# zengxiaofei/HapHiC

Hardware: NVIDIA H100
Metric: hic_pairs_per_sec_matrix_build (higher is better)
Workload: dtype int32 counts / fp32 matrix

## Files before the change

### haphic_b200/csrc/hh_common.cuh

```cuda
#pragma once

#include <cuda_runtime.h>
#include <stdint.h>
#include <stdio.h>
#include <stdarg.h>
#include <string.h>
#include <new>
#include <vector>

#include "../../include/haphic_b200.h"

void hh_set_error(const char* fmt, ...);

#define HH_CUDA(expr)                                                                         \
    do {                                                                                      \
        cudaError_t _e = (expr);                                                              \
        if (_e != cudaSuccess) {                                                              \
            hh_set_error("%s:%d: %s failed: %s", __FILE__, __LINE__, #expr, cudaGetErrorString(_e)); \
            return (_e == cudaErrorMemoryAllocation) ? HH_ERR_NOMEM : HH_ERR_CUDA;            \
        }                                                                                     \
    } while (0)

#define HH_CHECK(expr)                                                                        \
    do {                                                                                      \
        int _rc = (expr);                                                                     \
        if (_rc != HH_OK) return _rc;                                                         \
    } while (0)

#define HH_REQUIRE(cond, code, ...)                                                           \
    do {                                                                                      \
        if (!(cond)) {                                                                        \
            hh_set_error(__VA_ARGS__);                                                        \
            return (code);                                                                    \
        }                                                                                     \
    } while (0)

#define HH_LAUNCH(ctx, kernel, grid, block, smem, ...)                                        \
    do {                                                                                      \
        kernel<<<(grid), (block), (smem), (ctx)->stream>>>(__VA_ARGS__);                      \
        (ctx)->launches++;                                                                    \
        HH_CUDA(cudaGetLastError());                                                          \
    } while (0)

struct hh_ctx {
    int device;
    int sm_count;
    size_t smem_optin;
    size_t l2_bytes;
    cudaStream_t stream;
    int64_t launches;
    uint64_t* h_scratch;
    uint64_t* d_scratch;
    struct ws_block {
        void* p;
        size_t bytes;
        bool used;
        uint64_t tick;
    };
    std::vector<ws_block>* ws;
    uint64_t ws_tick;
};

void* hh_ws_alloc_bytes(hh_ctx* ctx, size_t bytes);
bool hh_ws_release(hh_ctx* ctx, void* p);
void hh_ws_free_ptr(hh_ctx* ctx, void* p);
template <typename T>
static inline int hh_ws_alloc(hh_ctx* ctx, T** p, size_t count) {
    *p = reinterpret_cast<T*>(hh_ws_alloc_bytes(ctx, (count ? count : 1) * sizeof(T)));
    return *p ? HH_OK : HH_ERR_NOMEM;
}
template <typename T>
static inline void hh_ws_free(hh_ctx* ctx, T*& p) {
    if (p) hh_ws_free_ptr(ctx, (void*)p);
    p = nullptr;
}

extern thread_local hh_ctx* hh_tls_ctx;
struct hh_scope {
    hh_ctx* prev;
    explicit hh_scope(hh_ctx* c) : prev(hh_tls_ctx) {
        hh_tls_ctx = c;
        if (c) cudaSetDevice(c->device);
    }
    ~hh_scope() { hh_tls_ctx = prev; }
};

#define HH_WS_MIN ((size_t)32 << 20)
template <typename T>
static inline int hh_dmalloc(T** p, size_t count) {
    *p = nullptr;
    if (count == 0) count = 1;
    if (hh_tls_ctx && count * sizeof(T) >= HH_WS_MIN) {
        *p = reinterpret_cast<T*>(hh_ws_alloc_bytes(hh_tls_ctx, count * sizeof(T)));
        return *p ? HH_OK : HH_ERR_NOMEM;
    }
    cudaError_t e = hh_tls_ctx ? cudaMallocAsync((void**)p, count * sizeof(T), hh_tls_ctx->stream)
                               : cudaMalloc((void**)p, count * sizeof(T));
    if (e != cudaSuccess) {
        hh_set_error("cudaMalloc of %zu bytes failed: %s", count * sizeof(T), cudaGetErrorString(e));
        cudaGetLastError();
        return HH_ERR_NOMEM;
    }
    return HH_OK;
}
template <typename T>
static inline void hh_dfree(T*& p) {
    if (p) {
        if (hh_ws_release(hh_tls_ctx, (void*)p)) {
        } else if (hh_tls_ctx) {
            cudaFreeAsync((void*)p, hh_tls_ctx->stream);
        } else {
            cudaFree((void*)p);
        }
    }
    p = nullptr;
}

#define HH_FULL_MASK 0xffffffffu

__device__ __forceinline__ int hh_lane() { return threadIdx.x & 31; }
__device__ __forceinline__ int hh_warp() { return threadIdx.x >> 5; }

__device__ __forceinline__ double hh_warp_sum(double v) {
#pragma unroll
    for (int o = 16; o > 0; o >>= 1) v += __shfl_xor_sync(HH_FULL_MASK, v, o);
    return v;
}
__device__ __forceinline__ int hh_warp_sum(int v) {
#pragma unroll
    for (int o = 16; o > 0; o >>= 1) v += __shfl_xor_sync(HH_FULL_MASK, v, o);
    return v;
}
__device__ __forceinline__ unsigned long long hh_warp_sum(unsigned long long v) {
#pragma unroll
    for (int o = 16; o > 0; o >>= 1) v += __shfl_xor_sync(HH_FULL_MASK, v, o);
    return v;
}
template <typename T>
__device__ __forceinline__ T hh_warp_incl_scan(T v) {
#pragma unroll
    for (int o = 1; o < 32; o <<= 1) {
        const T t = __shfl_up_sync(HH_FULL_MASK, v, o);
        if (hh_lane() >= o) v += t;
    }
    return v;
}
__device__ __forceinline__ float hh_warp_max(float v) {
#pragma unroll
    for (int o = 16; o > 0; o >>= 1) v = fmaxf(v, __shfl_xor_sync(HH_FULL_MASK, v, o));
    return v;
}

__device__ __forceinline__ int4 hh_ld_stream(const int4* p) {
    int4 r;
    asm volatile("ld.global.nc.L1::no_allocate.v4.s32 {%0, %1, %2, %3}, [%4];"
                 : "=r"(r.x), "=r"(r.y), "=r"(r.z), "=r"(r.w)
                 : "l"(p));
    return r;
}
__device__ __forceinline__ unsigned long long hh_ld_stream_u64(const unsigned long long* p) {
    unsigned long long r;
    asm volatile("ld.global.nc.L1::no_allocate.u64 %0, [%1];" : "=l"(r) : "l"(p));
    return r;
}
__device__ __forceinline__ float4 hh_ld_stream_f4(const float4* p) {
    float4 r;
    asm volatile("ld.global.nc.L1::no_allocate.v4.f32 {%0, %1, %2, %3}, [%4];"
                 : "=f"(r.x), "=f"(r.y), "=f"(r.z), "=f"(r.w)
                 : "l"(p));
    return r;
}

template <typename K>
static inline int hh_resident_grid(hh_ctx* ctx, K kernel, int threads, size_t smem, int* grid) {
    int per_sm = 0;
    HH_CUDA(cudaOccupancyMaxActiveBlocksPerMultiprocessor(&per_sm, kernel, threads, smem));
    HH_REQUIRE(per_sm > 0, HH_ERR_CUDA, "a kernel of %d threads and %zu bytes of shared memory does not fit an SM", threads, smem);
    *grid = ctx->sm_count * per_sm;
    return HH_OK;
}

__global__ void hh_k_scan_small(const int* __restrict__ in, int64_t* __restrict__ out, int n);
int hh_exclusive_scan_i32(hh_ctx* ctx, const int* d_in, int64_t* d_out, int n);
```

### haphic_b200/csrc/hh_links.cu

```cuda
#include "hh_common.cuh"
#include "hh_internal.cuh"
#include <cub/cub.cuh>
#include <stdlib.h>
#include <algorithm>
#include <vector>

#define HH_EMPTY_KEY 0xFFFFFFFFFFFFFFFFull
#define HH_NONE32 0xFFFFFFFFu

struct __align__(32) hh_slot {
    uint32_t first_full, first_flank, full, flank, ht, th, tt, pad;
};

struct hh_partset {
    void* buf;
    bool narrow;
    unsigned long long* cursor;
    uint64_t pcap;
    int64_t sized_for, sent;
};

struct hh_links {
    hh_ctx* ctx;
    int32_t n_ctg;
// ... 41 lines not shown
    int32_t* d_deg;
    int64_t n_pass;
    uint64_t gen;
    bool ix_valid;
    uint64_t ix_gen;
    int ix_normalize;
    double ix_w;
    std::vector<uint8_t> ix_keep;
    std::vector<int32_t> ix_hap;
    unsigned long long* d_ul_key = nullptr;
    int32_t* d_ul_slot = nullptr;
    int64_t n_ul = 0;
};

__device__ __forceinline__ uint64_t hh_mix64(uint64_t k) {
    k ^= k >> 33;
    k *= 0xff51afd7ed558ccdull;
    k ^= k >> 33;
    k *= 0xc4ceb9fe1a85ec53ull;
    k ^= k >> 33;
    return k;
}

__device__ __forceinline__ uint64_t hh_probe_insert(uint64_t* __restrict__ keys, uint64_t cap, uint64_t key, bool* inserted) {
    const uint64_t mask = cap - 1;
    uint64_t slot = hh_mix64(key) & mask;
    *inserted = false;
    for (uint64_t probes = 0; probes < cap; ++probes) {
        uint64_t k = *((volatile uint64_t*)(keys + slot));
        if (k == key) return slot;
        if (k == HH_EMPTY_KEY) {
            unsigned long long prev = atomicCAS((unsigned long long*)(keys + slot), (unsigned long long)HH_EMPTY_KEY,
                                                (unsigned long long)key);
            if (prev == HH_EMPTY_KEY) {
                *inserted = true;
                return slot;
            }
            if (prev == key) return slot;
        }
        slot = (slot + 1) & mask;
    }
    return cap;
}

__global__ void hh_k_links_init(uint64_t* __restrict__ keys, hh_slot* __restrict__ vals, uint64_t cap) {
    const uint64_t stride = (uint64_t)gridDim.x * blockDim.x;
    for (uint64_t s = (uint64_t)blockIdx.x * blockDim.x + threadIdx.x; s < cap; s += stride) {
        keys[s] = HH_EMPTY_KEY;
        uint4* v = reinterpret_cast<uint4*>(vals + s);
        v[0] = make_uint4(HH_NONE32, HH_NONE32, 0u, 0u);
        v[1] = make_uint4(0u, 0u, 0u, 0u);
    }
}

#define HH_F_FLANK 1u
#define HH_F_TI 2u
#define HH_F_TJ 4u

struct hh_pair {
    int a, b;
    unsigned flags;
};

__device__ __forceinline__ uint64_t hh_pair_key(int a, int b) { return ((uint64_t)(uint32_t)a << 32) | (uint64_t)(uint32_t)b; }

__device__ __forceinline__ void hh_swap_ends(int& a, int& b, int& pa, int& pb) {
    int t = a; a = b; b = t;
    t = pa; pa = pb; pb = t;
}

__device__ __forceinline__ void hh_pair_flags(int a, int b, int pa, int pb, const int32_t* __restrict__ ctg_len,
                                              const uint8_t* __restrict__ in_nx, int64_t flank_bp, hh_pair* out) {
    const int64_t coord_i = (int64_t)pa + 1, coord_j = (int64_t)pb + 1;
    const int64_t li = ctg_len[a], lj = ctg_len[b];
    const bool fi = (flank_bp == 0) || (coord_i <= flank_bp) || (coord_i > li - flank_bp);
    const bool fj = (flank_bp == 0) || (coord_j <= flank_bp) || (coord_j > lj - flank_bp);
    out->a = a;
    out->b = b;
    out->flags = ((fi && fj && in_nx[a] && in_nx[b]) ? HH_F_FLANK : 0u)
                 | ((coord_i * 2 > li) ? HH_F_TI : 0u) | ((coord_j * 2 > lj) ? HH_F_TJ : 0u);
}

__device__ __forceinline__ bool hh_classify_contig(int4 r, int32_t n_ctg, const int32_t* __restrict__ ctg_len,
                                                   const int32_t* __restrict__ name_rank, const uint8_t* __restrict__ in_nx,
                                                   int64_t flank_bp, hh_pair* out) {
    int a = r.x, b = r.z, pa = r.y, pb = r.w;
    if (a == b || (unsigned)a >= (unsigned)n_ctg || (unsigned)b >= (unsigned)n_ctg) return false;
    if (name_rank[a] > name_rank[b]) hh_swap_ends(a, b, pa, pb);
    hh_pair_flags(a, b, pa, pb, ctg_len, in_nx, flank_bp, out);
    return true;
}

__device__ __forceinline__ int64_t hh_floor_div(int64_t x, int64_t d) { return x >= 0 ? x / d : -((-x + d - 1) / d); }

__device__ __forceinline__ bool hh_to_bin(int& f, int& p, int nbins, int64_t bin_size) {
    const int64_t nb = ((int64_t)p + 1 + bin_size - 1) / bin_size;
    const bool exists = p >= 0 && nb >= 1 && nb <= (int64_t)nbins;
    f += (int)(nb - 1);
    p = (int)((int64_t)p - (nb - 1) * bin_size);
    return exists;
}

__device__ __forceinline__ bool hh_classify_frag(int4 r, int32_t n_src, const int32_t* __restrict__ src_rank,
                                                 const int32_t* __restrict__ fbase, int64_t bin_size, const int32_t* __restrict__ ctg_len,
                                                 const int32_t* __restrict__ name_rank, const uint8_t* __restrict__ in_nx,
                                                 int64_t flank_bp, uint32_t idx, unsigned long long* __restrict__ counters,
                                                 hh_pair* out) {
    int a = r.x, b = r.z, pa = r.y, pb = r.w;
    if ((unsigned)a >= (unsigned)n_src || (unsigned)b >= (unsigned)n_src) return false;
    if (a == b && fbase[a + 1] - fbase[a] <= 1) return false;
    if (src_rank[a] > src_rank[b] || (a == b && pa > pb)) hh_swap_ends(a, b, pa, pb);
    int fa = fbase[a], fb = fbase[b];
    const int na = fbase[a + 1] - fa, nb = fbase[b + 1] - fb;
    if (a == b && hh_floor_div((int64_t)pa, bin_size) == hh_floor_div((int64_t)pb, bin_size)) return false;
    bool bad = false;
    if (na > 1) bad = !hh_to_bin(fa, pa, na, bin_size);
    if (nb > 1) bad = !hh_to_bin(fb, pb, nb, bin_size) || bad;
    if (bad) {
        atomicAdd(counters + 5, 1ull);
        atomicMax(counters + 6, (unsigned long long)idx + 1ull);
        return false;
    }
    if (fa == fb) return false;
    if ((na > 1 || nb > 1) && name_rank[fa] > name_rank[fb]) hh_swap_ends(fa, fb, pa, pb);
    hh_pair_flags(fa, fb, pa, pb, ctg_len, in_nx, flank_bp, out);
    return true;
}

struct hh_group {
    bool leader;
    uint32_t first_all, first_flank;
    unsigned full, flank, ht, th, tt;
};

__device__ __forceinline__ hh_group hh_warp_fold(bool ok, uint64_t key, uint32_t idx, unsigned flags) {
    const int lane = threadIdx.x & 31;
    if (!ok) key = HH_EMPTY_KEY - 1 - (uint64_t)lane;
    const unsigned peers = __match_any_sync(HH_FULL_MASK, key);
    const bool fl = ok && (flags & HH_F_FLANK), ti = (flags & HH_F_TI) != 0, tj = (flags & HH_F_TJ) != 0;
    hh_group g;
    g.first_all = __reduce_min_sync(peers, ok ? idx : HH_NONE32);
    g.first_flank = __reduce_min_sync(peers, fl ? idx : HH_NONE32);
    const unsigned b_fl = __ballot_sync(HH_FULL_MASK, fl);
    const unsigned b_ht = __ballot_sync(HH_FULL_MASK, ok && !ti && tj);
    const unsigned b_th = __ballot_sync(HH_FULL_MASK, ok && ti && !tj);
    const unsigned b_tt = __ballot_sync(HH_FULL_MASK, ok && ti && tj);
    g.leader = ok && lane == (__ffs(peers) - 1);
    g.full = __popc(peers);
    g.flank = __popc(peers & b_fl);
    g.ht = __popc(peers & b_ht);
    g.th = __popc(peers & b_th);
    g.tt = __popc(peers & b_tt);
    return g;
}

__device__ __forceinline__ void hh_slot_update(hh_slot* v, const hh_group& g) {
    atomicAdd(&v->full, g.full);
    atomicMin(&v->first_full, g.first_all);
    if (g.flank) {
        atomicAdd(&v->flank, g.flank);
        atomicMin(&v->first_flank, g.first_flank);
    }
    if (g.ht) atomicAdd(&v->ht, g.ht);
    if (g.th) atomicAdd(&v->th, g.th);
    if (g.tt) atomicAdd(&v->tt, g.tt);
}

__device__ __forceinline__ void hh_entry_store(uint32_t* __restrict__ o, uint64_t key, uint32_t full, uint32_t flank, uint32_t first_full,
                                               uint32_t first_flank, uint32_t ht, uint32_t th, uint32_t tt) {
    o[HH_E_I] = (uint32_t)(key >> 32);
    o[HH_E_J] = (uint32_t)key;
    o[HH_E_FULL] = full;
    o[HH_E_FLANK] = flank;
    o[HH_E_FIRST_FULL] = first_full;
    o[HH_E_FIRST_FLANK] = first_flank;
    o[HH_E_HT] = ht;
    o[HH_E_TH] = th;
    o[HH_E_TT] = tt;
}

__device__ __forceinline__ void hh_entry_store(uint32_t* __restrict__ o, uint64_t key, uint4 v0, uint4 v1) {
    hh_entry_store(o, key, v0.z, v0.w, v0.x, v0.y, v1.x, v1.y, v1.z);
}

__device__ __forceinline__ unsigned int hh_block_rank(unsigned int cnt, unsigned int* s_wtot, unsigned int* total) {
    const int lane = threadIdx.x & 31, wv = threadIdx.x >> 5;
    unsigned int incl = cnt;
#pragma unroll
    for (int o = 1; o < 32; o <<= 1) {
        const unsigned int t = __shfl_up_sync(HH_FULL_MASK, incl, o);
        if (lane >= o) incl += t;
    }
    __syncthreads();
    if (lane == 31) s_wtot[wv] = incl;
    __syncthreads();
    unsigned int before = 0, all = 0;
#pragma unroll
    for (int k = 0; k < 8; ++k) {
        const unsigned int t = s_wtot[k];
        before += (k < wv) ? t : 0u;
        all += t;
    }
    *total = all;
    return before + incl - cnt;
}

__global__ void __launch_bounds__(256)
hh_k_links_insert(const int4* __restrict__ rec, int64_t n_rec, uint32_t stream_off, int32_t n_ctg,
                  const int32_t* __restrict__ ctg_len, const int32_t* __restrict__ name_rank,
                  const uint8_t* __restrict__ in_nx, int64_t flank_bp, uint64_t* __restrict__ keys,
                  hh_slot* __restrict__ vals, uint64_t cap, unsigned long long* __restrict__ ctg_links,
                  unsigned long long* __restrict__ counters, const int32_t* __restrict__ src_rank,
                  const int32_t* __restrict__ fbase, int64_t bin_size, int32_t n_src, const uint32_t* __restrict__ pos) {
    __shared__ unsigned int s_new, s_used, s_over;
    if (threadIdx.x == 0) {
        s_new = 0;
        s_used = 0;
        s_over = 0;
    }
    __syncthreads();
    const int lane = threadIdx.x & 31;
    const int64_t stride = (int64_t)gridDim.x * blockDim.x;
    unsigned int my_new = 0, my_used = 0;
    for (int64_t i0 = (int64_t)blockIdx.x * blockDim.x + (threadIdx.x - lane); i0 < n_rec; i0 += stride) {
        const int64_t i = i0 + lane;
        bool ok = i < n_rec;
        hh_pair p = {0, 0, 0u};
        uint32_t idx = HH_NONE32;
        if (ok) {
            const int4 r = hh_ld_stream(rec + i);
            idx = pos ? pos[i] : stream_off + (uint32_t)i;
            ok = fbase == nullptr ? hh_classify_contig(r, n_ctg, ctg_len, name_rank, in_nx, flank_bp, &p)
                                  : hh_classify_frag(r, n_src, src_rank, fbase, bin_size, ctg_len, name_rank, in_nx, flank_bp, idx,
                                                     counters, &p);
        }
        if (ok) my_used++;
        const uint64_t key = hh_pair_key(p.a, p.b);
        const hh_group g = hh_warp_fold(ok, key, idx, p.flags);
        if (g.leader) {
            bool inserted;
            const uint64_t slot = hh_probe_insert(keys, cap, key, &inserted);
            if (slot >= cap) {
                s_over = 1;
            } else {
                if (inserted) my_new++;
                hh_slot_update(vals + slot, g);
                if (g.flank) {
                    atomicAdd(ctg_links + p.a, (unsigned long long)g.flank);
                    atomicAdd(ctg_links + p.b, (unsigned long long)g.flank);
                }
            }
        }
    }
    if (my_new) atomicAdd(&s_new, my_new);
    if (my_used) atomicAdd(&s_used, my_used);
    __syncthreads();
    if (threadIdx.x == 0) {
        if (s_new) atomicAdd(counters + 0, (unsigned long long)s_new);
        if (s_used) atomicAdd(counters + 1, (unsigned long long)s_used);
        if (s_over) atomicExch(counters + 2, 1ull);
    }
}

#define HH_PART_TILE 4096
#define HH_PART_MAX 1024

#define HH_NREC_KBITS 16
#define HH_NREC_ZBITS 29
#define HH_NREC_ZEND (1ll << HH_NREC_ZBITS)

struct __align__(8) hh_nrec {
    unsigned long long v;
};

__device__ __forceinline__ int4 hh_ld_rec(const int4* p) { return hh_ld_stream(p); }
__device__ __forceinline__ hh_nrec hh_ld_rec(const hh_nrec* p) { return hh_nrec{hh_ld_stream_u64(&p->v)}; }

__device__ __forceinline__ uint32_t hh_rec_i(int4 r, int) { return (uint32_t)r.x; }
__device__ __forceinline__ uint32_t hh_rec_j(int4 r, int) { return (uint32_t)r.y; }
__device__ __forceinline__ uint32_t hh_rec_z(int4 r) { return (uint32_t)r.z; }
__device__ __forceinline__ unsigned hh_rec_flags(int4 r) { return (unsigned)r.w & 7u; }
__device__ __forceinline__ uint32_t hh_rec_i(hh_nrec r, int kbits) { return (uint32_t)(r.v >> 32) >> kbits; }
__device__ __forceinline__ uint32_t hh_rec_j(hh_nrec r, int kbits) { return (uint32_t)(r.v >> 32) & ((1u << kbits) - 1u); }
__device__ __forceinline__ uint32_t hh_rec_z(hh_nrec r) { return (uint32_t)r.v & (uint32_t)(HH_NREC_ZEND - 1); }
__device__ __forceinline__ unsigned hh_rec_flags(hh_nrec r) { return (uint32_t)r.v >> HH_NREC_ZBITS; }

__device__ __forceinline__ hh_nrec hh_nrec_make(uint32_t i, uint32_t j, uint32_t z, unsigned flags, int kbits) {
    return hh_nrec{((unsigned long long)((i << kbits) | j) << 32) | ((unsigned long long)flags << HH_NREC_ZBITS) | z};
}

__device__ __forceinline__ void hh_rec_put(int4* d, int4 s, int) { *d = s; }
__device__ __forceinline__ void hh_rec_put(hh_nrec* d, hh_nrec s, int) { *d = s; }
__device__ __forceinline__ void hh_rec_put(int4* d, hh_nrec s, int kbits) {
    *d = make_int4((int)hh_rec_i(s, kbits), (int)hh_rec_j(s, kbits), (int)hh_rec_z(s), (int)hh_rec_flags(s));
}
__device__ __forceinline__ void hh_rec_put(hh_nrec* d, int4 s, int kbits) {
    *d = hh_nrec_make(hh_rec_i(s, kbits), hh_rec_j(s, kbits), hh_rec_z(s), hh_rec_flags(s), kbits);
}

__device__ __forceinline__ void hh_rec_set_z(int4* r, uint32_t z) { r->z = (int)z; }
__device__ __forceinline__ void hh_rec_set_z(hh_nrec* r, uint32_t z) { r->v = (r->v & ~(unsigned long long)(HH_NREC_ZEND - 1)) | z; }

#define HH_STAGE_SMEM ((size_t)HH_PART_TILE * sizeof(int4))

__device__ __forceinline__ unsigned int hh_tile_scan(unsigned int* c, int n, unsigned int* s_wtot) {
    const int lane = threadIdx.x & 31, wv = threadIdx.x >> 5;
    const int per = (n + 511) >> 9, lo = threadIdx.x * per;
    __syncthreads();
    unsigned int sum = 0;
    for (int k = 0; k < per; ++k)
        if (lo + k < n) sum += c[lo + k];
    unsigned int incl = sum;
#pragma unroll
    for (int o = 1; o < 32; o <<= 1) {
        const unsigned int t = __shfl_up_sync(HH_FULL_MASK, incl, o);
        if (lane >= o) incl += t;
    }
    if (lane == 31) s_wtot[wv] = incl;
    __syncthreads();
    unsigned int run = incl - sum, all = 0;
#pragma unroll
    for (int k = 0; k < 16; ++k) {
        const unsigned int t = s_wtot[k];
        run += (k < wv) ? t : 0u;
        all += t;
    }
    for (int k = 0; k < per; ++k) {
        if (lo + k < n) {
            const unsigned int t = c[lo + k];
            c[lo + k] = run;
            run += t;
        }
    }
    __syncthreads();
    return all;
}

template <typename R>
__device__ __forceinline__ uint32_t hh_bucket_of(R r, int bucket_log, int kbits) {
    return (uint32_t)(hh_mix64(hh_pair_key((int)hh_rec_i(r, kbits), (int)hh_rec_j(r, kbits))) >> (64 - bucket_log));
}

__device__ __forceinline__ void hh_part_rec(int4* o, const hh_pair& pr, uint32_t z, unsigned p, int) {
    *o = make_int4(pr.a, pr.b, (int)z, (int)(pr.flags | (p << 8)));
}
__device__ __forceinline__ void hh_part_rec(hh_nrec* o, const hh_pair& pr, uint32_t z, unsigned, int kbits) {
    *o = hh_nrec_make((uint32_t)pr.a, (uint32_t)pr.b, z, pr.flags, kbits);
}
__device__ __forceinline__ unsigned hh_part_of(int4 r, int, int) { return (unsigned)r.w >> 8; }
__device__ __forceinline__ unsigned hh_part_of(hh_nrec r, int npart_log, int kbits) { return hh_bucket_of(r, npart_log, kbits); }

template <typename R>
__host__ __device__ constexpr int hh_scatter_tile() { return (int)(HH_STAGE_SMEM / sizeof(R)); }

template <typename R>
__global__ void __launch_bounds__(512, 2)
hh_k_part_scatter(const int4* __restrict__ rec, int64_t n_rec, uint32_t stream_off, int32_t n_ctg, const int32_t* __restrict__ ctg_len,
                  const int32_t* __restrict__ name_rank, const uint8_t* __restrict__ in_nx, int64_t flank_bp, int npart_log, int kbits,
                  R* __restrict__ pbuf, uint64_t pcap, unsigned long long* __restrict__ cursor, int4* __restrict__ spill,
                  uint64_t spill_cap, unsigned long long* __restrict__ spill_cursor, unsigned long long* __restrict__ counters) {
    constexpr int TILE = hh_scatter_tile<R>(), ITEMS = TILE / 512;
    extern __shared__ int4 s_stage_mem[];
    R* s_stage = reinterpret_cast<R*>(s_stage_mem);
    __shared__ unsigned int s_cnt[HH_PART_MAX];
    __shared__ unsigned long long s_base[HH_PART_MAX];
    __shared__ unsigned int s_wtot[16];
    __shared__ unsigned int s_used;
    const int npart = 1 << npart_log;
    const int64_t tiles = (n_rec + TILE - 1) / TILE;
    unsigned int my_used = 0;
    if (threadIdx.x == 0) s_used = 0;
    for (int64_t t = blockIdx.x; t < tiles; t += gridDim.x) {
        for (int k = threadIdx.x; k < npart; k += 512) s_cnt[k] = 0;
        __syncthreads();
        R out[ITEMS];
        uint32_t live = 0;
#pragma unroll
        for (int k = 0; k < ITEMS; ++k) {
            const int64_t i = t * TILE + (int64_t)k * 512 + threadIdx.x;
            if (i < n_rec) {
                hh_pair pr;
                if (hh_classify_contig(hh_ld_stream(rec + i), n_ctg, ctg_len, name_rank, in_nx, flank_bp, &pr)) {
                    const unsigned p = (unsigned)(hh_mix64(hh_pair_key(pr.a, pr.b)) >> (64 - npart_log));
                    hh_part_rec(&out[k], pr, (p << 13) | atomicAdd(&s_cnt[p], 1u), p, kbits);
                    live |= 1u << k;
                    my_used++;
                }
            }
        }
        __syncthreads();
        for (int k = threadIdx.x; k < npart; k += 512)
            if (s_cnt[k]) s_base[k] = atomicAdd(cursor + k, (unsigned long long)s_cnt[k]);
        const unsigned int n_tile = hh_tile_scan(s_cnt, npart, s_wtot);
#pragma unroll
        for (int k = 0; k < ITEMS; ++k) {
            if (!((live >> k) & 1u)) continue;
            const uint32_t at = hh_rec_z(out[k]);
            hh_rec_set_z(&out[k], stream_off + (uint32_t)(t * TILE + k * 512 + threadIdx.x));
            s_stage[s_cnt[at >> 13] + (at & 0x1FFFu)] = out[k];
        }
        __syncthreads();
        for (unsigned int e = threadIdx.x; e < n_tile; e += 512) {
            const R r = s_stage[e];
            const unsigned int p = hh_part_of(r, npart_log, kbits);
            const unsigned long long q = s_base[p] + (e - s_cnt[p]);
            if (q < pcap) {
                pbuf[(size_t)p * (size_t)pcap + (size_t)q] = r;
            } else {
                const unsigned long long sq = atomicAdd(spill_cursor, 1ull);
                if (sq < spill_cap) hh_rec_put(spill + sq, r, kbits);
                else atomicExch(counters + 2, 3ull);
            }
        }
        __syncthreads();
    }
    my_used = (unsigned)hh_warp_sum((int)my_used);
    if ((threadIdx.x & 31) == 0 && my_used) atomicAdd(&s_used, my_used);
    __syncthreads();
    if (threadIdx.x == 0 && s_used) atomicAdd(counters + 1, (unsigned long long)s_used);
}

#define HH_AGG_MEAN 2048
#define HH_SUB_MAX_LOG 12
#define HH_AGG_SLOTS 2048
#define HH_AGG_LIST (HH_AGG_SLOTS / 4 * 3)
#define HH_AGG_THREADS 256
#define HH_AGG_HOT 32

template <typename R>
__global__ void __launch_bounds__(512)
hh_k_part_hist(const R* __restrict__ pbuf, uint64_t pcap, const unsigned long long* __restrict__ cursor, int npart_log, int kbits,
               int64_t tpr, const int4* __restrict__ spill, int64_t n_spill, int bucket_log, unsigned int* __restrict__ bcnt) {
    constexpr int TILE = HH_PART_TILE, ITEMS = TILE / 512;
    __shared__ unsigned int s_cnt[1 << HH_SUB_MAX_LOG];
    const int sub_log = bucket_log - npart_log, nsub = 1 << sub_log;
    const int64_t region_tiles = ((int64_t)1 << npart_log) * tpr;
    const int64_t tiles = region_tiles + (n_spill + HH_PART_TILE - 1) / HH_PART_TILE;
    for (int64_t t = blockIdx.x; t < tiles; t += gridDim.x) {
        if (t >= region_tiles) {
            const int64_t base = (t - region_tiles) * HH_PART_TILE;
            for (int k = threadIdx.x; k < HH_PART_TILE; k += 512)
                if (base + k < n_spill) atomicAdd(bcnt + hh_bucket_of(hh_ld_rec(spill + base + k), bucket_log, kbits), 1u);
            continue;
        }
        const int p = (int)(t / tpr);
        const uint64_t start = (uint64_t)(t % tpr) * TILE;
        const uint64_t fill = min((uint64_t)cursor[p], pcap);
        if (start >= fill) continue;
        for (int k = threadIdx.x; k < nsub; k += 512) s_cnt[k] = 0;
        __syncthreads();
        const R* reg = pbuf + (size_t)p * (size_t)pcap;
#pragma unroll
        for (int k = 0; k < ITEMS; ++k) {
            const uint64_t i = start + (uint64_t)k * 512 + threadIdx.x;
            if (i < fill) atomicAdd(&s_cnt[hh_bucket_of(hh_ld_rec(reg + i), bucket_log, kbits) & (nsub - 1)], 1u);
        }
        __syncthreads();
        for (int k = threadIdx.x; k < nsub; k += 512)
            if (s_cnt[k]) atomicAdd(bcnt + ((size_t)p << sub_log) + k, s_cnt[k]);
        __syncthreads();
    }
}

template <typename R, typename D>
__global__ void __launch_bounds__(512, 2)
hh_k_part_scatter2(const R* __restrict__ pbuf, uint64_t pcap, const unsigned long long* __restrict__ cursor, int npart_log, int kbits,
                   int64_t tpr, const int4* __restrict__ spill, int64_t n_spill, int bucket_log, const int64_t* __restrict__ boff,
                   unsigned int* __restrict__ bfill, D* __restrict__ out, uint64_t n_out, unsigned long long* __restrict__ counters) {
    constexpr int TILE = HH_PART_TILE, ITEMS = TILE / 512;
    extern __shared__ int4 s_stage_mem[];
    R* s_stage = reinterpret_cast<R*>(s_stage_mem);
    __shared__ unsigned int s_cnt[1 << HH_SUB_MAX_LOG];
    __shared__ unsigned int s_base[1 << HH_SUB_MAX_LOG];
    __shared__ unsigned int s_wtot[16];
    const int sub_log = bucket_log - npart_log, nsub = 1 << sub_log;
    const int64_t region_tiles = ((int64_t)1 << npart_log) * tpr;
    const int64_t tiles = region_tiles + (n_spill + HH_PART_TILE - 1) / HH_PART_TILE;
    for (int64_t t = blockIdx.x; t < tiles; t += gridDim.x) {
        if (t >= region_tiles) {
            const int64_t base = (t - region_tiles) * HH_PART_TILE;
            for (int k = threadIdx.x; k < HH_PART_TILE; k += 512) {
                if (base + k >= n_spill) break;
                const int4 r = hh_ld_rec(spill + base + k);
                const uint32_t b = hh_bucket_of(r, bucket_log, kbits);
                const uint64_t q = (uint64_t)boff[b] + atomicAdd(bfill + b, 1u);
                if (q < n_out) hh_rec_put(out + q, r, kbits);
                else atomicExch(counters + 2, 6ull);
            }
            continue;
        }
        const int p = (int)(t / tpr);
        const uint64_t start = (uint64_t)(t % tpr) * TILE;
        const uint64_t fill = min((uint64_t)cursor[p], pcap);
        if (start >= fill) continue;
        for (int k = threadIdx.x; k < nsub; k += 512) s_cnt[k] = 0;
        __syncthreads();
        const R* reg = pbuf + (size_t)p * (size_t)pcap;
        R r[ITEMS];
        uint32_t at[ITEMS];
#pragma unroll
        for (int k = 0; k < ITEMS; ++k) {
            const uint64_t i = start + (uint64_t)k * 512 + threadIdx.x;
            at[k] = HH_NONE32;
            if (i < fill) {
                r[k] = hh_ld_rec(reg + i);
                const uint32_t sub = hh_bucket_of(r[k], bucket_log, kbits) & (nsub - 1);
                at[k] = (sub << 16) | atomicAdd(&s_cnt[sub], 1u);
            }
        }
        __syncthreads();
        for (int k = threadIdx.x; k < nsub; k += 512)
            if (s_cnt[k]) s_base[k] = atomicAdd(bfill + ((size_t)p << sub_log) + k, s_cnt[k]);
        const unsigned int n_tile = hh_tile_scan(s_cnt, nsub, s_wtot);
#pragma unroll
        for (int k = 0; k < ITEMS; ++k)
            if (at[k] != HH_NONE32) s_stage[s_cnt[at[k] >> 16] + (at[k] & 0xFFFFu)] = r[k];
        __syncthreads();
        for (unsigned int e = threadIdx.x; e < n_tile; e += 512) {
            const R rec = s_stage[e];
            const uint32_t sub = hh_bucket_of(rec, bucket_log, kbits) & (nsub - 1);
            const size_t b = ((size_t)p << sub_log) + sub;
            const uint64_t q = (uint64_t)boff[b] + s_base[sub] + (e - s_cnt[sub]);
            if (q < n_out) hh_rec_put(out + q, rec, kbits);
            else atomicExch(counters + 2, 6ull);
        }
        __syncthreads();
    }
}

#define HH_PK_FLANK 12
#define HH_PK_HT 24
#define HH_PK_TH 36
#define HH_PK_TT 48
#define HH_PK_MASK 0xFFFull
#define HH_PK_HEAD (1ull << 63)

struct hh_run {
    unsigned long long c;
    uint32_t first_full, first_flank;
};

struct hh_run_op {
    __device__ __forceinline__ hh_run operator()(const hh_run& a, const hh_run& b) const {
        if (b.c & HH_PK_HEAD) return b;
        return hh_run{a.c + b.c, min(a.first_full, b.first_full), min(a.first_flank, b.first_flank)};
    }
};

template <typename K>
__device__ __forceinline__ int hh_lower_bound(const K* a, int n, K k) {
    int lo = 0, hi = n;
    while (lo < hi) {
        const int mid = (lo + hi) >> 1;
        if (a[mid] < k) lo = mid + 1;
        else hi = mid;
    }
    return lo;
}

template <typename K, int ITEMS>
struct hh_bc_smem {
    typedef cub::BlockRadixSort<K, HH_AGG_THREADS, ITEMS, uint32_t> sort_t;
    typedef cub::BlockScan<hh_run, HH_AGG_THREADS> run_scan_t;
    typedef cub::BlockScan<unsigned int, HH_AGG_THREADS> cnt_scan_t;
    K key[HH_AGG_LIST];
    uint32_t val[HH_E_WORDS - 2][HH_AGG_LIST];
    uint32_t z[HH_AGG_THREADS * ITEMS];
    union {
        typename sort_t::TempStorage sort;
        struct {
            K first[HH_AGG_THREADS], last[HH_AGG_THREADS];
        } edge;
        K fresh[HH_AGG_THREADS * ITEMS];
    } u;
    typename run_scan_t::TempStorage run_scan;
    typename cnt_scan_t::TempStorage cnt_scan;
    unsigned long long base;
    int bucket;
};

template <typename K, int ITEMS, typename R>
__global__ void __launch_bounds__(HH_AGG_THREADS, 3)
hh_k_bucket_count(const R* __restrict__ rec, const int64_t* __restrict__ boff, int nbuckets, uint64_t hot, int kbits,
                  uint32_t* __restrict__ compact, uint64_t compact_cap, unsigned long long* __restrict__ ctg_links,
                  unsigned long long* __restrict__ counters, unsigned long long* __restrict__ agg, uint32_t* __restrict__ fallback) {
    typedef hh_bc_smem<K, ITEMS> smem_t;
    constexpr int S = HH_AGG_THREADS * ITEMS;
    extern __shared__ __align__(16) unsigned char hh_agg_smem[];
    smem_t& sm = *reinterpret_cast<smem_t*>(hh_agg_smem);
    const int t = threadIdx.x;
    const K jmask = ((K)1 << kbits) - 1;
    const hh_run none = {HH_PK_HEAD, HH_NONE32, HH_NONE32};
    unsigned int nfl = 0, n_done = 0;
    for (;;) {
        __syncthreads();
        if (t == 0) sm.bucket = (int)atomicAdd(agg + 0, 1ull);
        __syncthreads();
        const int bk = sm.bucket;
        if (bk >= nbuckets) break;
        const int64_t lo = boff[bk], n = boff[bk + 1] - lo;
        if ((uint64_t)n > hot) {
            if (t == 0) fallback[atomicAdd(agg + 1, 1ull)] = (uint32_t)bk;
            continue;
        }
        int tsize = HH_AGG_THREADS;
        while (tsize < HH_AGG_SLOTS && (int64_t)tsize * 2 < n * 3) tsize <<= 1;
        const int limit = tsize / 4 * 3;
        int na = 0;
        bool abandon = false;
        for (int64_t c0 = 0; c0 < n; c0 += S) {
            const int m = (int)min((int64_t)S, n - c0);
            K key[ITEMS];
            uint32_t pay[ITEMS];
            __syncthreads();
#pragma unroll
            for (int q = 0; q < ITEMS; ++q) {
                const int l = q * HH_AGG_THREADS + t;
                key[q] = ~(K)0;
                pay[q] = 0;
                if (l < m) {
                    const R r = hh_ld_rec(rec + lo + c0 + l);
                    key[q] = ((K)hh_rec_i(r, kbits) << kbits) | (K)hh_rec_j(r, kbits);
                    pay[q] = (uint32_t)l | (hh_rec_flags(r) << 11);
                    sm.z[l] = hh_rec_z(r);
                }
            }
            typename smem_t::sort_t(sm.u.sort).Sort(key, pay, 0, 2 * kbits);
            __syncthreads();
            sm.u.edge.first[t] = key[0];
            sm.u.edge.last[t] = key[ITEMS - 1];
            __syncthreads();
            const K prev = t > 0 ? sm.u.edge.last[t - 1] : ~(K)0;
            const K next = t + 1 < HH_AGG_THREADS ? sm.u.edge.first[t + 1] : ~(K)0;
            auto item = [&](int q) -> hh_run {
                const int pos = t * ITEMS + q;
                if (pos >= m) return none;
                const unsigned f = (pay[q] >> 11) & 7u;
                const uint32_t z = sm.z[pay[q] & 0x7FFu];
                const bool fl = f & HH_F_FLANK, ti = f & HH_F_TI, tj = f & HH_F_TJ;
// ... 1615 lines not shown
```

### haphic_b200/csrc/hh_matrix.cu

```cuda
#include "hh_common.cuh"
#include "hh_internal.cuh"
#include <algorithm>

__global__ void hh_k_set_tail(const int32_t* __restrict__ tail, int n_tail, int n_linked, const uint8_t* __restrict__ keep,
                              int32_t* __restrict__ index, int n_ctg, int* __restrict__ err) {
    int t = blockIdx.x * blockDim.x + threadIdx.x;
    if (t >= n_tail) return;
    const int c = tail[t];
    if (c < 0 || c >= n_ctg || !keep[c] || index[c] >= 0) {
        atomicExch(err, 1);
        return;
    }
    index[c] = n_linked + t;
}

__global__ void hh_k_check_index(const int32_t* __restrict__ index, const uint8_t* __restrict__ keep, int n_ctg, int n,
                                 int* __restrict__ err) {
    int c = blockIdx.x * blockDim.x + threadIdx.x;
    if (c >= n_ctg) return;
    const int ix = index[c];
    if (keep[c] ? (ix < 0 || ix >= n) : (ix >= 0)) atomicExch(err, 2);
}

__global__ void hh_k_fill_i32(int* __restrict__ p, int v, int n) {
    int i = blockIdx.x * blockDim.x + threadIdx.x;
    if (i < n) p[i] = v;
}

__global__ void hh_k_mat_colcnt(const int32_t* __restrict__ index, const int32_t* __restrict__ deg, int n_ctg, int self_loop,
                                int* __restrict__ colcnt) {
    const int c = blockIdx.x * blockDim.x + threadIdx.x;
    if (c >= n_ctg) return;
    const int ix = index[c];
    if (ix >= 0) colcnt[ix] = deg[c] + self_loop;
}

__global__ void hh_k_mat_self_loops(int n, const int64_t* __restrict__ colptr, int32_t* __restrict__ row, float* __restrict__ val) {
    const int c = blockIdx.x * blockDim.x + threadIdx.x;
    if (c >= n) return;
    const int64_t q = colptr[c];
    row[q] = c;
    val[q] = 1.0f;
}

__global__ void hh_k_mat_scatter(const uint32_t* __restrict__ compact, int64_t nnz, const int32_t* __restrict__ index,
                                 const unsigned long long* __restrict__ ctg_tot, int normalize, const int32_t* __restrict__ hap,
                                 double w, const int32_t* __restrict__ ul_path, const int32_t* __restrict__ ul_parent,
                                 const int64_t* __restrict__ colptr, int* __restrict__ cursor,
                                 int32_t* __restrict__ row, float* __restrict__ val) {
    const int64_t stride = (int64_t)gridDim.x * blockDim.x;
    for (int64_t e = (int64_t)blockIdx.x * blockDim.x + threadIdx.x; e < nnz; e += stride) {
        const uint32_t* p = compact + e * HH_E_WORDS;
        if (p[HH_E_FLANK] == 0) continue;
        const int ii = index[p[HH_E_I]], jj = index[p[HH_E_J]];
        if (ii < 0 || jj < 0) continue;
        double x;
        if (!hh_flank_value(p, ctg_tot, normalize, hap, w, ul_path, ul_parent, &x)) continue;
        const float v = (float)x;
        int64_t q = colptr[jj] + atomicAdd(cursor + jj, 1);
        row[q] = ii;
        val[q] = v;
        q = colptr[ii] + atomicAdd(cursor + ii, 1);
        row[q] = jj;
        val[q] = v;
    }
}

static int matrix_alloc(hh_ctx* ctx, int32_t n, int64_t nnz, hh_matrix** out) {
    hh_matrix* m = new (std::nothrow) hh_matrix();
    HH_REQUIRE(m != nullptr, HH_ERR_NOMEM, "hh_matrix: out of host memory");
    memset(m, 0, sizeof(*m));
    m->ctx = ctx;
    m->n = n;
    m->nnz = nnz;
    int rc;
    if ((rc = hh_dmalloc(&m->d_colptr, (size_t)n + 1)) != HH_OK || (rc = hh_dmalloc(&m->d_row, (size_t)nnz)) != HH_OK ||
        (rc = hh_dmalloc(&m->d_val, (size_t)nnz)) != HH_OK) {
        hh_matrix_destroy(m);
        return rc;
    }
    *out = m;
    return HH_OK;
}

extern "C" int hh_matrix_from_links(hh_links* lk, const uint8_t* keep, const int32_t* tail, int32_t n_tail,
                                    int normalize_by_nlinks, int add_self_loops, hh_matrix** out) {
    return hh_matrix_from_links_phased(lk, keep, tail, n_tail, normalize_by_nlinks, add_self_loops, nullptr, 0.0, out);
}

extern "C" int hh_matrix_from_links_phased(hh_links* lk, const uint8_t* keep, const int32_t* tail, int32_t n_tail,
                                           int normalize_by_nlinks, int add_self_loops, const int32_t* hap, double w,
                                           hh_matrix** out) {
    return hh_matrix_from_links_ex(lk, keep, tail, n_tail, normalize_by_nlinks, add_self_loops, hap, w, nullptr, nullptr, out);
}

extern "C" int hh_matrix_from_links_ex(hh_links* lk, const uint8_t* keep, const int32_t* tail, int32_t n_tail, int normalize_by_nlinks,
                                       int add_self_loops, const int32_t* hap, double w, const int32_t* ul_path,
                                       const int32_t* ul_parent, hh_matrix** out) {
    HH_REQUIRE(lk && keep && out, HH_ERR_ARG, "hh_matrix_from_links: NULL argument");
    hh_scope _scope(hh_links_ctx(lk));
    HH_REQUIRE(n_tail >= 0 && (tail || n_tail == 0), HH_ERR_ARG, "hh_matrix_from_links: bad tail");
    HH_REQUIRE(!ul_path == !ul_parent, HH_ERR_ARG, "hh_matrix_from_links_ex: give both ul_path and ul_parent, or neither");
    HH_REQUIRE(hh_links_finished(lk), HH_ERR_STATE, "hh_matrix_from_links: call hh_links_finish first");
    *out = nullptr;
    hh_ctx* ctx = hh_links_ctx(lk);
    HH_CUDA(cudaSetDevice(ctx->device));
    const int n_ctg = hh_links_n_ctg(lk);
    int32_t n_linked = 0;
    HH_CHECK(hh_links_linked_index_phased(lk, keep, normalize_by_nlinks, hap, w, nullptr, &n_linked));
    const int32_t* d_hap = hh_links_hap_dev(lk);
    const int32_t* d_index = hh_links_index_dev(lk, &n_linked);
    int64_t n_pass = 0;
    const int32_t* d_deg = hh_links_degree_dev(lk, &n_pass);
    const uint8_t* d_keep = hh_links_keep_dev(lk);
    HH_REQUIRE(n_tail <= n_ctg - n_linked, HH_ERR_ARG,
               "hh_matrix_from_links: tail lists an id that is dropped, linked, repeated or out of range");
    const int n = n_linked + n_tail;
    HH_REQUIRE(n > 0, HH_ERR_ARG, "hh_matrix_from_links: empty fragment set");
    const int sl = add_self_loops ? 1 : 0;
    const int64_t nnz = 2 * n_pass + (int64_t)sl * n;
    int* d_err = reinterpret_cast<int*>(ctx->d_scratch + 10);
    int32_t* d_tail = nullptr;
    int32_t* d_ul = nullptr;
    int* d_cnt = nullptr;
    hh_matrix* m = nullptr;
    int rc = [&]() -> int {
        HH_CHECK(matrix_alloc(ctx, n, nnz, &m));
        HH_CHECK(hh_dmalloc(&m->d_index, (size_t)n_ctg));
        m->n_index = n_ctg;
        HH_CUDA(cudaMemcpyAsync(m->d_index, d_index, (size_t)n_ctg * sizeof(int32_t), cudaMemcpyDeviceToDevice, ctx->stream));
        HH_CUDA(cudaMemsetAsync(d_err, 0, sizeof(int), ctx->stream));
        if (n_tail) {
            HH_CHECK(hh_dmalloc(&d_tail, (size_t)n_tail));
            HH_CUDA(cudaMemcpyAsync(d_tail, tail, (size_t)n_tail * sizeof(int32_t), cudaMemcpyHostToDevice, ctx->stream));
            HH_LAUNCH(ctx, hh_k_set_tail, (n_tail + 255) / 256, 256, 0, d_tail, n_tail, n_linked, d_keep, m->d_index, n_ctg, d_err);
        }
        HH_LAUNCH(ctx, hh_k_check_index, (n_ctg + 255) / 256, 256, 0, m->d_index, d_keep, n_ctg, n, d_err);
        HH_CHECK(hh_dmalloc(&d_cnt, (size_t)n));
        HH_LAUNCH(ctx, hh_k_fill_i32, (n + 255) / 256, 256, 0, d_cnt, sl, n);
        HH_LAUNCH(ctx, hh_k_mat_colcnt, (n_ctg + 255) / 256, 256, 0, d_index, d_deg, n_ctg, sl, d_cnt);
        HH_CHECK(hh_exclusive_scan_i32(ctx, d_cnt, m->d_colptr, n));
        int* d_cursor = d_cnt;
        HH_LAUNCH(ctx, hh_k_fill_i32, (n + 255) / 256, 256, 0, d_cursor, sl, n);
        if (sl) HH_LAUNCH(ctx, hh_k_mat_self_loops, (n + 255) / 256, 256, 0, n, m->d_colptr, m->d_row, m->d_val);
        int64_t nnz_c = 0;
        const uint32_t* compact = hh_links_compact(lk, &nnz_c);
        if (ul_path && n_pass) {
            HH_CHECK(hh_dmalloc(&d_ul, (size_t)n_ctg * 2));
            HH_CUDA(cudaMemcpyAsync(d_ul, ul_path, (size_t)n_ctg * sizeof(int32_t), cudaMemcpyHostToDevice, ctx->stream));
            HH_CUDA(cudaMemcpyAsync(d_ul + n_ctg, ul_parent, (size_t)n_ctg * sizeof(int32_t), cudaMemcpyHostToDevice, ctx->stream));
        }
        if (n_pass) {
            int gridc = 0;
            HH_CHECK(hh_resident_grid(ctx, hh_k_mat_scatter, 256, 0, &gridc));
            gridc = (int)std::min<int64_t>((nnz_c + 255) / 256, gridc);
            HH_LAUNCH(ctx, hh_k_mat_scatter, gridc, 256, 0, compact, nnz_c, d_index, hh_links_ctg_totals(lk), normalize_by_nlinks, d_hap,
                      w, d_ul, d_ul ? d_ul + n_ctg : nullptr, m->d_colptr, d_cursor, m->d_row, m->d_val);
        }
        HH_CUDA(cudaMemcpyAsync(ctx->h_scratch + 10, d_err, sizeof(int), cudaMemcpyDeviceToHost, ctx->stream));
        HH_CUDA(cudaStreamSynchronize(ctx->stream));
        const int err = *reinterpret_cast<int*>(ctx->h_scratch + 10);
        HH_REQUIRE(err == 0, HH_ERR_ARG,
                   err == 1 ? "hh_matrix_from_links: tail lists an id that is dropped, linked, repeated or out of range"
                            : "hh_matrix_from_links: keep mask and tail do not cover the fragment set exactly");
        return HH_OK;
    }();
    hh_dfree(d_tail);
    hh_dfree(d_ul);
    hh_dfree(d_cnt);
    if (rc != HH_OK) {
        hh_matrix_destroy(m);
        return rc;
    }
    *out = m;
    return HH_OK;
}

extern "C" int hh_matrix_from_csc(hh_ctx* ctx, int32_t n, const int64_t* indptr, const int32_t* indices, const float* data,
                                  hh_matrix** out) {
    HH_REQUIRE(ctx && indptr && out, HH_ERR_ARG, "hh_matrix_from_csc: NULL argument");
    hh_scope _scope(ctx);
    HH_REQUIRE(n > 0, HH_ERR_ARG, "hh_matrix_from_csc: n must be positive");
    *out = nullptr;
    HH_REQUIRE(indptr[0] == 0, HH_ERR_ARG, "hh_matrix_from_csc: indptr[0] must be 0");
    for (int32_t c = 0; c < n; ++c)
        HH_REQUIRE(indptr[c + 1] >= indptr[c] && indptr[c + 1] - indptr[c] <= n, HH_ERR_ARG,
                   "hh_matrix_from_csc: column %d has an invalid extent", c);
    const int64_t nnz = indptr[n];
    HH_REQUIRE(nnz == 0 || (indices && data), HH_ERR_ARG, "hh_matrix_from_csc: NULL indices/data");
    for (int64_t e = 0; e < nnz; ++e)
        HH_REQUIRE(indices[e] >= 0 && indices[e] < n, HH_ERR_ARG, "hh_matrix_from_csc: row index out of range at entry %lld",
                   (long long)e);
    HH_CUDA(cudaSetDevice(ctx->device));
    hh_matrix* m = nullptr;
    HH_CHECK(matrix_alloc(ctx, n, nnz, &m));
    int rc = [&]() -> int {
        HH_CUDA(cudaMemcpyAsync(m->d_colptr, indptr, ((size_t)n + 1) * sizeof(int64_t), cudaMemcpyHostToDevice, ctx->stream));
        if (nnz) {
            HH_CUDA(cudaMemcpyAsync(m->d_row, indices, (size_t)nnz * sizeof(int32_t), cudaMemcpyHostToDevice, ctx->stream));
            HH_CUDA(cudaMemcpyAsync(m->d_val, data, (size_t)nnz * sizeof(float), cudaMemcpyHostToDevice, ctx->stream));
        }
        HH_CUDA(cudaStreamSynchronize(ctx->stream));
        return HH_OK;
    }();
    if (rc != HH_OK) {
        hh_matrix_destroy(m);
        return rc;
    }
    *out = m;
    return HH_OK;
}

extern "C" int hh_matrix_info(hh_matrix* m, int32_t* n, int64_t* nnz) {
    HH_REQUIRE(m != nullptr, HH_ERR_ARG, "hh_matrix_info: NULL handle");
    if (n) *n = m->n;
    if (nnz) *nnz = m->nnz;
    return HH_OK;
}

extern "C" int hh_matrix_destroy(hh_matrix* m) {
    if (!m) return HH_OK;
    hh_scope _scope(m->ctx);
    cudaSetDevice(m->ctx->device);
    cudaStreamSynchronize(m->ctx->stream);
    hh_dfree(m->d_colptr);
    hh_dfree(m->d_row);
    hh_dfree(m->d_val);
    hh_dfree(m->d_index);
    delete m;
    return HH_OK;
}
```

Measured before the change: 6.366 billion.

## Replace atomic CSC scatter with two-pass group-bucketed staging and per-chunk placement

```diff
diff --git a/haphic_b200/csrc/hh_common.cuh b/haphic_b200/csrc/hh_common.cuh
--- a/haphic_b200/csrc/hh_common.cuh
+++ b/haphic_b200/csrc/hh_common.cuh
@@ -171,6 +171,39 @@
     return r;
 }
 
+__device__ __forceinline__ unsigned int hh_tile_scan(unsigned int* c, int n, unsigned int* s_wtot) {
+    const int lane = threadIdx.x & 31, wv = threadIdx.x >> 5;
+    const int per = (n + 511) >> 9, lo = threadIdx.x * per;
+    __syncthreads();
+    unsigned int sum = 0;
+    for (int k = 0; k < per; ++k)
+        if (lo + k < n) sum += c[lo + k];
+    unsigned int incl = sum;
+#pragma unroll
+    for (int o = 1; o < 32; o <<= 1) {
+        const unsigned int t = __shfl_up_sync(HH_FULL_MASK, incl, o);
+        if (lane >= o) incl += t;
+    }
+    if (lane == 31) s_wtot[wv] = incl;
+    __syncthreads();
+    unsigned int run = incl - sum, all = 0;
+#pragma unroll
+    for (int k = 0; k < 16; ++k) {
+        const unsigned int t = s_wtot[k];
+        run += (k < wv) ? t : 0u;
+        all += t;
+    }
+    for (int k = 0; k < per; ++k) {
+        if (lo + k < n) {
+            const unsigned int t = c[lo + k];
+            c[lo + k] = run;
+            run += t;
+        }
+    }
+    __syncthreads();
+    return all;
+}
+
 template <typename K>
 static inline int hh_resident_grid(hh_ctx* ctx, K kernel, int threads, size_t smem, int* grid) {
     int per_sm = 0;
diff --git a/haphic_b200/csrc/hh_links.cu b/haphic_b200/csrc/hh_links.cu
--- a/haphic_b200/csrc/hh_links.cu
+++ b/haphic_b200/csrc/hh_links.cu
@@ -367,39 +367,6 @@
 __device__ __forceinline__ void hh_rec_set_z(hh_nrec* r, uint32_t z) { r->v = (r->v & ~(unsigned long long)(HH_NREC_ZEND - 1)) | z; }
 
 #define HH_STAGE_SMEM ((size_t)HH_PART_TILE * sizeof(int4))
-
-__device__ __forceinline__ unsigned int hh_tile_scan(unsigned int* c, int n, unsigned int* s_wtot) {
-    const int lane = threadIdx.x & 31, wv = threadIdx.x >> 5;
-    const int per = (n + 511) >> 9, lo = threadIdx.x * per;
-    __syncthreads();
-    unsigned int sum = 0;
-    for (int k = 0; k < per; ++k)
-        if (lo + k < n) sum += c[lo + k];
-    unsigned int incl = sum;
-#pragma unroll
-    for (int o = 1; o < 32; o <<= 1) {
-        const unsigned int t = __shfl_up_sync(HH_FULL_MASK, incl, o);
-        if (lane >= o) incl += t;
-    }
-    if (lane == 31) s_wtot[wv] = incl;
-    __syncthreads();
-    unsigned int run = incl - sum, all = 0;
-#pragma unroll
-    for (int k = 0; k < 16; ++k) {
-        const unsigned int t = s_wtot[k];
-        run += (k < wv) ? t : 0u;
-        all += t;
-    }
-    for (int k = 0; k < per; ++k) {
-        if (lo + k < n) {
-            const unsigned int t = c[lo + k];
-            c[lo + k] = run;
-            run += t;
-        }
-    }
-    __syncthreads();
-    return all;
-}
 
 template <typename R>
 __device__ __forceinline__ uint32_t hh_bucket_of(R r, int bucket_log, int kbits) {
diff --git a/haphic_b200/csrc/hh_matrix.cu b/haphic_b200/csrc/hh_matrix.cu
--- a/haphic_b200/csrc/hh_matrix.cu
+++ b/haphic_b200/csrc/hh_matrix.cu
@@ -43,26 +43,168 @@
     val[q] = 1.0f;
 }
 
-__global__ void hh_k_mat_scatter(const uint32_t* __restrict__ compact, int64_t nnz, const int32_t* __restrict__ index,
-                                 const unsigned long long* __restrict__ ctg_tot, int normalize, const int32_t* __restrict__ hap,
-                                 double w, const int32_t* __restrict__ ul_path, const int32_t* __restrict__ ul_parent,
-                                 const int64_t* __restrict__ colptr, int* __restrict__ cursor,
-                                 int32_t* __restrict__ row, float* __restrict__ val) {
-    const int64_t stride = (int64_t)gridDim.x * blockDim.x;
-    for (int64_t e = (int64_t)blockIdx.x * blockDim.x + threadIdx.x; e < nnz; e += stride) {
-        const uint32_t* p = compact + e * HH_E_WORDS;
-        if (p[HH_E_FLANK] == 0) continue;
-        const int ii = index[p[HH_E_I]], jj = index[p[HH_E_J]];
-        if (ii < 0 || jj < 0) continue;
-        double x;
-        if (!hh_flank_value(p, ctg_tot, normalize, hap, w, ul_path, ul_parent, &x)) continue;
-        const float v = (float)x;
-        int64_t q = colptr[jj] + atomicAdd(cursor + jj, 1);
-        row[q] = ii;
-        val[q] = v;
-        q = colptr[ii] + atomicAdd(cursor + ii, 1);
-        row[q] = jj;
-        val[q] = v;
+#define HH_MAT_TILE 4096
+#define HH_MAT_CHUNK 8192
+#define HH_MAT_MAX_N (1 << 22)
+
+struct hh_mat_chunk {
+    long long start;
+    int len;
+    int group;
+};
+
+static int hh_mat_cbits(int n) {
+    int bits = 0;
+    while (((int64_t)1 << bits) < n) ++bits;
+    return std::max(8, bits - 12);
+}
+
+static size_t hh_mat_group_smem(int ngroups) {
+    return (size_t)2 * HH_MAT_TILE * (sizeof(uint2) + sizeof(uint16_t)) + (size_t)ngroups * (sizeof(unsigned long long) + sizeof(unsigned int));
+}
+
+__global__ void __launch_bounds__(512, 2)
+hh_k_mat_group(const uint32_t* __restrict__ compact, int64_t nnz, const int32_t* __restrict__ index,
+               const unsigned long long* __restrict__ ctg_tot, int normalize, const int32_t* __restrict__ hap, double w,
+               const int32_t* __restrict__ ul_path, const int32_t* __restrict__ ul_parent, int cbits, int ngroups,
+               unsigned long long* __restrict__ gcur, uint2* __restrict__ stage) {
+    constexpr int ITEMS = HH_MAT_TILE / 512;
+    extern __shared__ uint2 s_mat_mem[];
+    uint2* s_stage = s_mat_mem;
+    uint16_t* s_grp = reinterpret_cast<uint16_t*>(s_stage + 2 * HH_MAT_TILE);
+    unsigned long long* s_base = reinterpret_cast<unsigned long long*>(s_grp + 2 * HH_MAT_TILE);
+    unsigned int* s_cnt = reinterpret_cast<unsigned int*>(s_base + ngroups);
+    __shared__ unsigned int s_wtot[16];
+    const uint32_t cmask = (1u << cbits) - 1u;
+    const int64_t tiles = (nnz + HH_MAT_TILE - 1) / HH_MAT_TILE;
+    for (int64_t t = blockIdx.x; t < tiles; t += gridDim.x) {
+        for (int k = threadIdx.x; k < ngroups; k += 512) s_cnt[k] = 0;
+        __syncthreads();
+        int ii[ITEMS], jj[ITEMS];
+        float v[ITEMS];
+#pragma unroll
+        for (int k = 0; k < ITEMS; ++k) {
+            const int64_t e = t * HH_MAT_TILE + (int64_t)k * 512 + threadIdx.x;
+            ii[k] = -1;
+            if (e < nnz) {
+                const uint32_t* p = compact + e * HH_E_WORDS;
+                const uint32_t fl = p[HH_E_FLANK], ci = p[HH_E_I], cj = p[HH_E_J];
+                if (fl) {
+                    ii[k] = (int)ci;
+                    jj[k] = (int)cj;
+                }
+            }
+        }
+#pragma unroll
+        for (int k = 0; k < ITEMS; ++k) {
+            if (ii[k] < 0) continue;
+            ii[k] = index[ii[k]];
+            jj[k] = index[jj[k]];
+        }
+#pragma unroll
+        for (int k = 0; k < ITEMS; ++k) {
+            if (ii[k] < 0 || jj[k] < 0) {
+                ii[k] = -1;
+                continue;
+            }
+            double x;
+            if (!hh_flank_value(compact + (t * HH_MAT_TILE + (int64_t)k * 512 + threadIdx.x) * HH_E_WORDS, ctg_tot, normalize, hap,
+                                w, ul_path, ul_parent, &x)) {
+                ii[k] = -1;
+                continue;
+            }
+            v[k] = (float)x;
+            atomicAdd(&s_cnt[jj[k] >> cbits], 1u);
+            atomicAdd(&s_cnt[ii[k] >> cbits], 1u);
+        }
+        __syncthreads();
+        for (int k = threadIdx.x; k < ngroups; k += 512)
+            if (s_cnt[k]) s_base[k] = atomicAdd(gcur + k, (unsigned long long)s_cnt[k]);
+        const unsigned int n_tile = hh_tile_scan(s_cnt, ngroups, s_wtot);
+        for (int k = threadIdx.x; k < ngroups; k += 512) s_base[k] -= s_cnt[k];
+        __syncthreads();
+#pragma unroll
+        for (int k = 0; k < ITEMS; ++k) {
+            if (ii[k] < 0) continue;
+            const uint32_t a = (uint32_t)ii[k], b = (uint32_t)jj[k];
+            const unsigned int qa = atomicAdd(&s_cnt[b >> cbits], 1u);
+            s_stage[qa] = make_uint2(a << cbits | (b & cmask), __float_as_uint(v[k]));
+            s_grp[qa] = (uint16_t)(b >> cbits);
+            const unsigned int qb = atomicAdd(&s_cnt[a >> cbits], 1u);
+            s_stage[qb] = make_uint2(b << cbits | (a & cmask), __float_as_uint(v[k]));
+            s_grp[qb] = (uint16_t)(a >> cbits);
+        }
+        __syncthreads();
+        for (unsigned int e = threadIdx.x; e < n_tile; e += 512) stage[s_base[s_grp[e]] + e] = s_stage[e];
+        __syncthreads();
+    }
+}
+
+__global__ void __launch_bounds__(512)
+hh_k_mat_chunks(const int64_t* __restrict__ colptr, int n, int cbits, int ngroups, int sl, unsigned long long* __restrict__ gcur,
+                hh_mat_chunk* __restrict__ chunk, unsigned int* __restrict__ n_chunks) {
+    __shared__ unsigned int s_off[4096];
+    __shared__ unsigned int s_wtot[16];
+    for (int g = threadIdx.x; g < ngroups; g += 512) {
+        const int lo = g << cbits, hi = min(n, lo + (1 << cbits));
+        const int64_t s = colptr[lo] + (int64_t)sl * (hi - lo);
+        gcur[g] = (unsigned long long)s;
+        s_off[g] = (unsigned int)((colptr[hi] - s + HH_MAT_CHUNK - 1) / HH_MAT_CHUNK);
+    }
+    const unsigned int total = hh_tile_scan(s_off, ngroups, s_wtot);
+    for (unsigned int c = threadIdx.x; c < total; c += 512) {
+        int g = 0;
+        for (int step = 2048; step > 0; step >>= 1)
+            if (g + step < ngroups && s_off[g + step] <= c) g += step;
+        const int lo = g << cbits, hi = min(n, lo + (1 << cbits));
+        const int64_t s = colptr[lo] + (int64_t)sl * (hi - lo) + (int64_t)(c - s_off[g]) * HH_MAT_CHUNK;
+        chunk[c] = hh_mat_chunk{s, (int)min((int64_t)HH_MAT_CHUNK, colptr[hi] - s), g};
+    }
+    if (threadIdx.x == 0) *n_chunks = total;
+}
+
+__global__ void __launch_bounds__(512, 2)
+hh_k_mat_place(const uint2* __restrict__ stage, const hh_mat_chunk* __restrict__ chunk, const unsigned int* __restrict__ n_chunks,
+               int cbits, const int64_t* __restrict__ colptr, int* __restrict__ cursor, int32_t* __restrict__ row,
+               float* __restrict__ val) {
+    constexpr int ITEMS = HH_MAT_CHUNK / 512;
+    extern __shared__ uint2 s_mat_mem[];
+    uint2* s_rec = s_mat_mem;
+    __shared__ unsigned int s_cnt[1024];
+    __shared__ long long s_base[1024];
+    __shared__ unsigned int s_wtot[16];
+    const int ncol = 1 << cbits;
+    const uint32_t cmask = (uint32_t)ncol - 1u;
+    const unsigned int total = *n_chunks;
+    for (unsigned int c = blockIdx.x; c < total; c += gridDim.x) {
+        const hh_mat_chunk ch = chunk[c];
+        for (int k = threadIdx.x; k < ncol; k += 512) s_cnt[k] = 0;
+        __syncthreads();
+        uint2 r[ITEMS];
+#pragma unroll
+        for (int k = 0; k < ITEMS; ++k)
+            if (k * 512 + (int)threadIdx.x < ch.len) r[k] = stage[ch.start + k * 512 + threadIdx.x];
+#pragma unroll
+        for (int k = 0; k < ITEMS; ++k)
+            if (k * 512 + (int)threadIdx.x < ch.len) atomicAdd(&s_cnt[r[k].x & cmask], 1u);
+        __syncthreads();
+        const int col0 = ch.group << cbits;
+        for (int k = threadIdx.x; k < ncol; k += 512)
+            if (s_cnt[k]) s_base[k] = colptr[col0 + k] + atomicAdd(cursor + col0 + k, (int)s_cnt[k]);
+        hh_tile_scan(s_cnt, ncol, s_wtot);
+        for (int k = threadIdx.x; k < ncol; k += 512) s_base[k] -= s_cnt[k];
+        __syncthreads();
+#pragma unroll
+        for (int k = 0; k < ITEMS; ++k)
+            if (k * 512 + (int)threadIdx.x < ch.len) s_rec[atomicAdd(&s_cnt[r[k].x & cmask], 1u)] = r[k];
+        __syncthreads();
+        for (int e = threadIdx.x; e < ch.len; e += 512) {
+            const uint2 x = s_rec[e];
+            const long long q = s_base[x.x & cmask] + e;
+            row[q] = (int32_t)(x.x >> cbits);
+            val[q] = __uint_as_float(x.y);
+        }
+        __syncthreads();
     }
 }
 
@@ -117,12 +259,18 @@
                "hh_matrix_from_links: tail lists an id that is dropped, linked, repeated or out of range");
     const int n = n_linked + n_tail;
     HH_REQUIRE(n > 0, HH_ERR_ARG, "hh_matrix_from_links: empty fragment set");
+    HH_REQUIRE(n <= HH_MAT_MAX_N, HH_ERR_ARG, "hh_matrix_from_links: %d fragments in the matrix, at most %d are supported", n,
+               HH_MAT_MAX_N);
     const int sl = add_self_loops ? 1 : 0;
     const int64_t nnz = 2 * n_pass + (int64_t)sl * n;
     int* d_err = reinterpret_cast<int*>(ctx->d_scratch + 10);
     int32_t* d_tail = nullptr;
     int32_t* d_ul = nullptr;
     int* d_cnt = nullptr;
+    uint2* d_stage = nullptr;
+    unsigned long long* d_gcur = nullptr;
+    hh_mat_chunk* d_chunk = nullptr;
+    unsigned int* d_nchunk = nullptr;
     hh_matrix* m = nullptr;
     int rc = [&]() -> int {
         HH_CHECK(matrix_alloc(ctx, n, nnz, &m));
@@ -151,11 +299,25 @@
             HH_CUDA(cudaMemcpyAsync(d_ul + n_ctg, ul_parent, (size_t)n_ctg * sizeof(int32_t), cudaMemcpyHostToDevice, ctx->stream));
         }
         if (n_pass) {
-            int gridc = 0;
-            HH_CHECK(hh_resident_grid(ctx, hh_k_mat_scatter, 256, 0, &gridc));
-            gridc = (int)std::min<int64_t>((nnz_c + 255) / 256, gridc);
-            HH_LAUNCH(ctx, hh_k_mat_scatter, gridc, 256, 0, compact, nnz_c, d_index, hh_links_ctg_totals(lk), normalize_by_nlinks, d_hap,
-                      w, d_ul, d_ul ? d_ul + n_ctg : nullptr, m->d_colptr, d_cursor, m->d_row, m->d_val);
+            const int cbits = hh_mat_cbits(n), ngroups = (n + (1 << cbits) - 1) >> cbits;
+            const int64_t max_chunks = (nnz + HH_MAT_CHUNK - 1) / HH_MAT_CHUNK + ngroups;
+            HH_CHECK(hh_ws_alloc(ctx, &d_stage, (size_t)nnz));
+            HH_CHECK(hh_dmalloc(&d_gcur, (size_t)ngroups));
+            HH_CHECK(hh_dmalloc(&d_chunk, (size_t)max_chunks));
+            HH_CHECK(hh_dmalloc(&d_nchunk, 1));
+            HH_LAUNCH(ctx, hh_k_mat_chunks, 1, 512, 0, m->d_colptr, n, cbits, ngroups, sl, d_gcur, d_chunk, d_nchunk);
+            const size_t smem1 = hh_mat_group_smem(ngroups), smem2 = (size_t)HH_MAT_CHUNK * sizeof(uint2);
+            int grid = 0;
+            HH_CUDA(cudaFuncSetAttribute(hh_k_mat_group, cudaFuncAttributeMaxDynamicSharedMemorySize, (int)smem1));
+            HH_CHECK(hh_resident_grid(ctx, hh_k_mat_group, 512, smem1, &grid));
+            grid = (int)std::min<int64_t>((nnz_c + HH_MAT_TILE - 1) / HH_MAT_TILE, grid);
+            HH_LAUNCH(ctx, hh_k_mat_group, grid, 512, smem1, compact, nnz_c, d_index, hh_links_ctg_totals(lk), normalize_by_nlinks,
+                      d_hap, w, d_ul, d_ul ? d_ul + n_ctg : nullptr, cbits, ngroups, d_gcur, d_stage);
+            HH_CUDA(cudaFuncSetAttribute(hh_k_mat_place, cudaFuncAttributeMaxDynamicSharedMemorySize, (int)smem2));
+            HH_CHECK(hh_resident_grid(ctx, hh_k_mat_place, 512, smem2, &grid));
+            grid = (int)std::min<int64_t>(max_chunks, grid);
+            HH_LAUNCH(ctx, hh_k_mat_place, grid, 512, smem2, d_stage, d_chunk, d_nchunk, cbits, m->d_colptr, d_cursor, m->d_row,
+                      m->d_val);
         }
         HH_CUDA(cudaMemcpyAsync(ctx->h_scratch + 10, d_err, sizeof(int), cudaMemcpyDeviceToHost, ctx->stream));
         HH_CUDA(cudaStreamSynchronize(ctx->stream));
@@ -168,6 +330,10 @@
     hh_dfree(d_tail);
     hh_dfree(d_ul);
     hh_dfree(d_cnt);
+    hh_ws_free(ctx, d_stage);
+    hh_dfree(d_gcur);
+    hh_dfree(d_chunk);
+    hh_dfree(d_nchunk);
     if (rc != HH_OK) {
         hh_matrix_destroy(m);
         return rc;
```

New measurement: 7.558 billion (median of 6 runs). +18.7%, better.
